# vaenyr/stable-diffusion-on-device

Measured on AMD Instinct MI355X. Metric: images/sec + per-UNet-step ms, SD v1.4 512x512 20-step PLMS, 1/2/4/8 MI355X, higher is better.
Workload: dtype f16; 1 GPU; SD v1.4 txt2img 512x512, 20-step PLMS (21 UNet evals, batch 2 = cond+uncond per image), CLIP encode + VAE decode + uint8, guidance 7.5; images_per_gpu=1, global_batch=1, parallelism=dp1 (image shards, 1 RCCL broadcast), hip_graph=True, trajectory_graph=True, decode_overlaps_next_sampling=False

## Files before the change

include/sdod_hip.h:

```cpp
#ifndef SDOD_HIP_H
#define SDOD_HIP_H

#include <stddef.h>
#include <stdint.h>

#ifndef SDOD_API
#define SDOD_API
#endif

#ifdef __cplusplus
extern "C" {
#endif

enum sdod_act { SDOD_ACT_NONE = 0, SDOD_ACT_SILU = 1, SDOD_ACT_GELU = 2, SDOD_ACT_QUICK_GELU = 3 };
enum sdod_dtype { SDOD_F16 = 0, SDOD_F32 = 1, SDOD_U8Q = 2, SDOD_BF16 = 3  };
enum sdod_a_mode { SDOD_A_ROWS = 0, SDOD_A_CONV3X3 = 1  };

typedef struct sdod_gemm_desc {
    const void* a;
    const void* a2;
    const void* w;
    const void* bias;
    const void* row_bias;
    const void* residual;
// ... 71 lines not shown
    size_t slab_floats;
    const void* bias;
    const void* bias2;
    const void* row_bias;
    int ld_row_bias;
    const void* residual;
    int ldr;
    void* x_out;
    float alpha;
    int act;
    int M, N;
} sdod_gn_reduce;
SDOD_API int sdod_gemm_reduce_info(const sdod_gemm_desc* d, sdod_gn_reduce* out);
SDOD_API int sdod_group_norm_reduce_ok(int hw, int c0, int c1, int groups);
SDOD_API int sdod_group_norm_reduce_nhwc(const sdod_gn_reduce* red, const void* x2, void* y, const float* weight,
                                         const float* bias, int n, int hw, int c0, int c1, int groups, float eps, int silu,
                                         void* stream);

SDOD_API int sdod_ln_fold_f16(void* w, int n, int k, int ldw, const float* gamma, const float* beta, const float* bias_in,
                              float* s_out, float* t_out, void* stream);
SDOD_API int sdod_compose_linear_f16(const void* p, int ldp, const void* w, int ldw, void* c, int ldc, int n_out, int n_mid, int k,
                                     const float* bias_w, const float* bias_p, float* bias_out, void* stream);
SDOD_API int sdod_layer_norm_f16(const void* x, void* y, const float* weight, const float* bias, int m, int c,
                                 float eps, void* stream);

SDOD_API int sdod_attention_f16(const void* q, const void* k, const void* v, void* out, int batch, int heads,
                                int lq, int lk, int d, int ldq, int ldk, int ldv, int ldo, float scale, int causal,
                                void* stream);

SDOD_API int sdod_xattn_fold_f16(const void* kv, int ld_kv, int k_off, int v_off, int n_img, int L, const void* wq, int ldq,
                                 const void* sq, const void* tq, const void* wo, int ldwo, int heads, int d, float scale, void* w1,
                                 void* s1, void* t1, void* w2, void* stream);

SDOD_API int sdod_softmax_rows_f16(const void* x, void* y, int m, int n, void* stream);

SDOD_API int sdod_geglu_f16(const void* x, void* y, int m, int c, void* stream);
SDOD_API int sdod_act_f16(const void* x, void* y, size_t n, int act, void* stream);
SDOD_API int sdod_add_f16(const void* a, const void* b, void* y, size_t n, void* stream);
SDOD_API int sdod_concat_channels_f16(const void* a, const void* b, void* y, size_t rows, int c0, int c1, void* stream);
SDOD_API int sdod_im2col3x3_small_f16(const void* x, void* y, int n_img, int h, int w, int c, int kpad, void* stream);
SDOD_API int sdod_latent_im2col_f16(const float* x, void* y, int n_img, int h, int w, int c, int kpad, float scale, void* stream);

SDOD_API int sdod_conv_in_f16(const float* x, const void* w, const float* bias, void* y, int n_img, int h, int wd, int c, int cout,
                              float scale, void* stream);
SDOD_API int sdod_image_conv_in_f16(const uint8_t* img, const void* w, const float* bias, void* y, int n_img, int h, int wd, int cout,
                                    void* stream);
SDOD_API int sdod_encode_latent_f32(const float* moments, const float* n1, const float* n2, float* x, float* z0, int n, int c, int hw,
                                    float sqrt_at, float sqrt_one_minus_at, uint64_t seed, uint64_t image_index0, void* stream);
SDOD_API int sdod_nchw_f32_to_nhwc_f16(const float* x, void* y, int n, int c, int hw, float scale, void* stream);
SDOD_API int sdod_latent_prep_f16(const float* x, const float* w, const float* b, void* y, int n, int c, int hw,
                                  float scale, void* stream);
SDOD_API int sdod_nhwc_f16_to_nchw_f32(const void* x, float* y, int n, int c, int hw, void* stream);
SDOD_API int sdod_embedding_f16(const int32_t* ids, const void* table, const void* pos, void* y, int rows, int seq,
                                int c, void* stream);
SDOD_API int sdod_timestep_features_f16(const float* t, void* y, int n, int dim, void* stream);

SDOD_API int sdod_stage_unet_inputs(const float* x, float* x_dst, size_t lat_count, int reps, const void* temb_row,
                                    void* temb_dst, size_t temb_width, int temb_reps, void* stream);
SDOD_API int sdod_randn_f32(float* out, uint32_t* words_out, size_t count, uint64_t seed, uint64_t stream_id, void* stream);

SDOD_API int sdod_cfg_combine(const void* eps_nhwc, float* e_out, int n, int c, int hw, float guidance,
                              int uncond_first, int mode, void* stream);
SDOD_API int sdod_dpm_update(float* x, const float* eps, float* y_prev, size_t count, int order, float sigma_s,
                             float alpha_s, float sigma_ratio, float c_prev, float c_cur, void* stream);
SDOD_API int sdod_ddim_step_f32(float* x, const float* e, size_t count, float sqrt_one_minus_at, float sqrt_at,
                                float sqrt_a_prev, float dir_coef, void* stream);
// ... 40 lines not shown
```

stable-diffusion-on-device_amd/csrc/gemm.hip:

```cpp
#include "common.h"
#include "sdod_hip.h"
#include "host_util.h"

#include <algorithm>
#include <cmath>
#include <cstdlib>
#include <type_traits>

namespace {

struct GemmP {
    const f16* a0;
    const f16* a1;
    const f16* w;
    const float* bias;
    const f16* row_bias;
    const f16* residual;
    f16* out;
    float* partial;
    int M, N, K;
    int lda, ldw, ldo, ldr;
    int mode;
    int h_in, w_in, h_out, w_out, c0, c1, stride, ups, ksize;
    int pad;
// ... 1131 lines not shown
                            acc[i][j][r] = e;
                            sum += e;
                        }
                    sum = quad_rows_sum(sum);
                    const float inv = __builtin_amdgcn_rcpf(sum);
#pragma unroll
                    for (int j = 0; j < TN; ++j)
#pragma unroll
                        for (int r = 0; r < 4; ++r) acc[i][j][r] *= inv;
                }
            }
        }
#pragma unroll
        for (int i = 0; i < TM; ++i) {
            const int ml = wm * WTM + i * 16 + e_m;
#pragma unroll
            for (int j = 0; j < TN; ++j) {
                const int nl = wn * WTN + j * 16 + e_n;
                f16x4 h;
#pragma unroll
                for (int r = 0; r < 4; ++r) h[r] = (f16)acc[i][j][r];
                *reinterpret_cast<f16x4*>(sC + ml * SC + nl) = h;
            }
        }
    }
    __syncthreads();
    STAMP(3);

    store_phase();
#ifdef SDOD_GEMM_STAMP
    wait_vmcnt<0>();
    STAMP(4);
#endif
}

template <int BM, int BN, int WM, int WN, int STAGES>
__global__ __launch_bounds__(768) void gemm_apanel_kernel(const GemmP p, const f16* __restrict__ zeros) {
    constexpr int NL = 4;
    constexpr int WTM = BM / WM, WTN = BN / WN;
    constexpr int TM = WTM / 16, TN = WTN / 16;
    constexpr int A_LD = BM / (8 * NL), B_LD = BN / (8 * NL);
    constexpr int AHEAD = STAGES - 1;
    constexpr int ASLAB = BM * 64, WSLAB = BN * 64;
    static_assert(WM * WN == 4 && BM % 32 == 0 && BN % 64 == 0 && BN <= 128 && TM >= 1 && TN >= 2 && TN % 2 == 0, "tile shape");
    static_assert(B_LD * AHEAD + 2 < 64, "vmcnt is a 6-bit counter");

    extern __shared__ __attribute__((aligned(16))) char smem_raw[];
    const int KT = p.K / BK;
    f16* sAp = reinterpret_cast<f16*>(smem_raw);
    f16* sW = sAp + (size_t)KT * ASLAB;
    float* colv = reinterpret_cast<float*>(sW + (size_t)STAGES * WSLAB);
    float* ln_stats = colv + 6 * BN;

    const int tid = threadIdx.x;
    const int lane = tid & 63;
    const int wave = __builtin_amdgcn_readfirstlane(tid >> 6);

    const int lid = xcd_remap(blockIdx.x, (int)gridDim.x);
    int pm, ng;
    if (p.ap_nmajor) {
        ng = lid / p.ap_panels;
        pm = lid - ng * p.ap_panels;
    } else {
        pm = lid / p.ap_groups;
        ng = lid - pm * p.ap_groups;
    }
// ... 1759 lines not shown
    hipStream_t st = (hipStream_t)stream;
    int rc = sdod_gemm_f16(d, stream);
    if (rc) return rc;
    hipEvent_t ev[32];
    for (int i = 0; i < 2 * iters; ++i) SDOD_HIP_CHECK(hipEventCreate(&ev[i]));
    float* sink = (float*)scratch;
    const size_t a_bytes = d->a_mode == SDOD_A_ROWS ? (size_t)d->M * d->lda * 2 : (size_t)d->n_img * d->h_in * d->w_in * d->c0 * 2;
    for (int i = 0; i < iters; ++i) {
        SDOD_LAUNCH(cache_sweep_kernel, dim3(2048), dim3(256), 0, st, (float4*)scratch, scratch_bytes / 16);
        touch(d->a, a_bytes, sink, st);
        if (d->a2 && d->c1) touch(d->a2, (size_t)d->n_img * d->h_in * d->w_in * d->c1 * 2, sink, st);
        if (d->residual) touch(d->residual, (size_t)d->M * d->ldr * 2, sink, st);
        if (d->t0 && d->k_tail) touch(d->t0, (size_t)d->M * d->tc0 * 2, sink, st);
        if (d->t1 && d->k_tail && d->tc1) touch(d->t1, (size_t)d->M * d->tc1 * 2, sink, st);
        SDOD_HIP_CHECK(hipEventRecord(ev[2 * i], st));
        rc = sdod_gemm_f16(d, stream);
        if (rc) return rc;
        SDOD_HIP_CHECK(hipEventRecord(ev[2 * i + 1], st));
    }
    SDOD_HIP_CHECK(hipEventSynchronize(ev[2 * iters - 1]));
    float tot = 0.f, best = 1e30f;
    for (int i = 0; i < iters; ++i) {
        float ms = 0.f;
        SDOD_HIP_CHECK(hipEventElapsedTime(&ms, ev[2 * i], ev[2 * i + 1]));
        tot += ms;
        best = ms < best ? ms : best;
    }
    for (int i = 0; i < 2 * iters; ++i) (void)hipEventDestroy(ev[i]);
    *ms_avg = tot / iters;
    if (ms_min) *ms_min = best;
    return 0;
    SDOD_CATCH
}
```

stable-diffusion-on-device_amd/csrc/graphs.hip:

```cpp
#include "engine.h"

namespace sdod {

static void check_rc2(int rc) {
    if (rc != 0) throw Error(rc, get_last_error());
}

int Graph::group_first(const std::string& group) const {
    auto it = gindex_.find(group);
    if (it == gindex_.end()) throw Error(INTERNAL_ERROR, "unknown parameter group " + group);
    return groups_[it->second].front();
}

const char* Graph::group_base(const std::string& group) const {
    auto it = gindex_.find(group);
    if (it == gindex_.end()) throw Error(INTERNAL_ERROR, "unknown parameter group " + group);
    return params_[groups_[it->second].front()].dev;
}

Act Graph::res_block(const std::string& pfx, const Act& x, const Act* x2, int cout, const f16* emb_all, int emb_ld, int& emb_off) {
    const int cin = x.c + (x2 ? x2->c : 0);
    quant_rows(x.rows());
    const int n1w = P(pfx + ".in_layers.0.weight", {cin}, PK_VEC), n1b = P(pfx + ".in_layers.0.bias", {cin}, PK_VEC);
    const int c1w = P(pfx + ".in_layers.2.weight", {cout, cin, 3, 3}, PK_CONV3), c1b = P(pfx + ".in_layers.2.bias", {cout}, PK_VEC);
// ... 82 lines not shown
    const bool compose = compose_on && !quant_block;
    int f2w, pow_;
    if (compose) {
        f2w = Pc(tb + ".ff.net.2.weight", {C, 4 * C}, PK_LINEAR, 5 * C, 0, -1);
        pow_ = lin ? Pc(pfx + ".proj_out.weight", {C, C}, PK_LINEAR, 5 * C, 4 * C, f2w)
                   : Pc(pfx + ".proj_out.weight", {C, C, 1, 1}, PK_CONV1, 5 * C, 4 * C, f2w);
    } else {
        f2w = P(tb + ".ff.net.2.weight", {C, 4 * C}, PK_LINEAR);
        pow_ = lin ? P(pfx + ".proj_out.weight", {C, C}, PK_LINEAR) : P(pfx + ".proj_out.weight", {C, C, 1, 1}, PK_CONV1);
    }
    const int f2b = P(tb + ".ff.net.2.bias", {C}, PK_VEC);
    const int pob = P(pfx + ".proj_out.bias", {C}, PK_VEC);
    if (mode_ == DECLARE) return act(x.n, x.h, x.w, C);

    Act g = group_norm(x, nullptr, nw, nb, 1e-6f, false);
    Act t0 = act(B, 1, L, C);
    { GemmOpt o; o.bias = pib; linear(g.p, rows, C, piw, C, t0.p, o); }
    release(g);
    const bool fold = !quant_block;
    auto normed = [&](const Act& src, int lw, int lb) -> Act { return layer_norm(src, lw, lb, 1e-5f); };
    f16* qkv = alloc((size_t)rows * 3 * C);
    if (fold) {
        GemmOpt o; o.ln_w = l1w; o.ln_b = l1b;
        linear_raw(t0.p, rows, C, reinterpret_cast<const f16*>(group_base(gq)), C, 3 * C, qkv, o);
    } else {
        Act nrm = normed(t0, l1w, l1b);
        GemmOpt o; o.wq_scale = qscale_of(group_first(gq)); o.wq_off = qoff_of(group_first(gq));
        linear_raw(nrm.p, rows, C, reinterpret_cast<const f16*>(group_base(gq)), C, 3 * C, qkv, o);
        release(nrm);
    }
    f16* a1 = alloc((size_t)rows * C);
    attention(qkv, qkv + C, qkv + 2 * C, a1, B, heads, L, L, d, 3 * C, 3 * C, 3 * C, C, false);
    release(qkv);
    Act t1 = act(B, 1, L, C);
    { GemmOpt o; o.bias = o1b; o.residual = t0.p; linear(a1, rows, C, o1w, C, t1.p, o); }
    release(a1); release(t0);
    static const bool xfold_on = [] { const char* e = std::getenv("SDOD_XATTN_FOLD"); return !(e && e[0] == '0'); }();
    const int NK = heads * 80;
    const bool xfold = xfold_on && fold && ctx.w <= 80 && NK % 320 == 0 && L % 32 == 0 && d <= 160 && d % 4 == 0;
    if (xfold) {
        f16 *w1 = nullptr, *w2 = nullptr;
        float *s1 = nullptr, *t1v = nullptr;
        f16* wq = reinterpret_cast<f16*>(params_[q2w].dev);
        const f16* wo = reinterpret_cast<const f16*>(params_[o2w].dev);
        if (mode_ == REAL) {
            SDOD_HIP_CHECK(hipMalloc((void**)&w1, (size_t)B * NK * C * sizeof(f16)));
            SDOD_HIP_CHECK(hipMalloc((void**)&w2, (size_t)B * NK * C * sizeof(f16)));
            SDOD_HIP_CHECK(hipMalloc((void**)&s1, (size_t)B * NK * sizeof(float)));
            SDOD_HIP_CHECK(hipMalloc((void**)&t1v, (size_t)B * NK * sizeof(float)));
            derived_.push_back(w1); derived_.push_back(w2); derived_.push_back(s1); derived_.push_back(t1v);
            const LnVecs qv = ln_fold_vectors(wq, C, C, C, l2w, l2b, nullptr);
            const f16* kvp = kv_all_;
            const int ldkv = kv_total_, koff = my_kv, Lk = ctx.w, hh = heads, dd = d;
            const float scale = 1.0f / sqrtf((float)d);
            to_static_ = true;
            sink().push_back(Op{[=](hipStream_t st) {
                check_rc2(sdod_xattn_fold_f16(kvp, ldkv, koff, koff + C, B, Lk, wq, C, qv.s, qv.t, wo, C, hh, dd, scale, w1, s1, t1v, w2, st));
            }, "xattn_fold", 4.0 * B * NK * (double)C * d, 4.0 * B * NK * C * 2, "C" + std::to_string(C) + " d" + std::to_string(d)});
            to_static_ = false;
        }
        const f16* w1p = mode_ == REAL ? w1 : wq;
        const f16* w2p = mode_ == REAL ? w2 : wq;
        f16* pb = alloc((size_t)rows * NK);
        { GemmOpt o; o.ln_s_raw = mode_ == REAL ? s1 : reinterpret_cast<const float*>(wq); o.bias_raw = mode_ == REAL ? t1v : reinterpret_cast<const float*>(wq);
          o.w_img_stride = NK * C; o.vec_img_stride = NK; o.softmax_cols = 80; o.rows_per_img = L;
          linear_raw(t1.p, rows, C, w1p, C, NK, pb, o); }
        GemmOpt o2;
        o2.bias = o2b; o2.residual = t1.p; o2.w_img_stride = C * NK; o2.rows_per_img = L;
        if (compose) {
            f16* cat = alloc((size_t)rows * 5 * C);
            f16* t2c = cat + 4 * C;
            o2.ldr = C; o2.ldo = 5 * C;
            linear_raw(pb, rows, NK, w2p, NK, C, t2c, o2);
            release(pb); release(t1);
            { GemmOpt o; o.bias = f1b; o.geglu = true; o.ln_w = l3w; o.ln_b = l3b; o.lda = 5 * C; o.ldo = 5 * C; linear(t2c, rows, C, f1w, 8 * C, cat, o); }
            float* bc = nullptr;
            if (mode_ == REAL) {
                SDOD_HIP_CHECK(hipMalloc((void**)&bc, (size_t)C * sizeof(float)));
                derived_.push_back(bc);
                f16* wc = reinterpret_cast<f16*>(params_[f2w].dev);
                compose_jobs_.push_back(ComposeJob{wc, wc + 4 * C, 5 * C, C, C, 4 * C, W<float>(f2b), W<float>(pob), bc});
            }
            Act out = act(x.n, x.h, x.w, C);
            { GemmOpt o; o.bias_raw = mode_ == REAL ? bc : reinterpret_cast<const float*>(params_[f2w].dev); o.residual = x.p;
              linear_raw(cat, rows, 5 * C, reinterpret_cast<const f16*>(params_[f2w].dev), 5 * C, C, out.p, o); }
            release(cat);
            return out;
        }
        Act t2 = act(B, 1, L, C);
        linear_raw(pb, rows, NK, w2p, NK, C, t2.p, o2);
        release(pb); release(t1);
        f16* gg = alloc((size_t)rows * 4 * C);
        { GemmOpt o; o.bias = f1b; o.geglu = true; o.ln_w = l3w; o.ln_b = l3b; linear(t2.p, rows, C, f1w, 8 * C, gg, o); }
        Act t3 = act(B, 1, L, C);
        { GemmOpt o; o.bias = f2b; o.residual = t2.p; linear(gg, rows, 4 * C, f2w, C, t3.p, o); }
        release(gg); release(t2);
        Act out = act(x.n, x.h, x.w, C);
        { GemmOpt o; o.bias = pob; o.residual = x.p; linear(t3.p, rows, C, pow_, C, out.p, o); }
        release(t3);
        return out;
    }
    f16* q2 = alloc((size_t)rows * C);
    if (fold) {
        GemmOpt o; o.ln_w = l2w; o.ln_b = l2b; linear(t1.p, rows, C, q2w, C, q2, o);
    } else {
        Act nrm = normed(t1, l2w, l2b);
        linear(nrm.p, rows, C, q2w, C, q2, GemmOpt{});
        release(nrm);
    }
    const int Lk = ctx.w;
    const f16* kv = kv_all_ + my_kv;
    f16* a2 = alloc((size_t)rows * C);
    attention(q2, kv, kv + C, a2, B, heads, L, Lk, d, C, kv_total_, kv_total_, C, false);
    release(q2);
    if (compose) {
        f16* cat = alloc((size_t)rows * 5 * C);
        f16* t2c = cat + 4 * C;
        { GemmOpt o; o.bias = o2b; o.residual = t1.p; o.ldr = C; o.ldo = 5 * C; linear(a2, rows, C, o2w, C, t2c, o); }
        release(a2); release(t1);
        { GemmOpt o; o.bias = f1b; o.geglu = true; o.ln_w = l3w; o.ln_b = l3b; o.lda = 5 * C; o.ldo = 5 * C; linear(t2c, rows, C, f1w, 8 * C, cat, o); }
        float* bc = nullptr;
        if (mode_ == REAL) {
            SDOD_HIP_CHECK(hipMalloc((void**)&bc, (size_t)C * sizeof(float)));
            derived_.push_back(bc);
            f16* wc = reinterpret_cast<f16*>(params_[f2w].dev);
            compose_jobs_.push_back(ComposeJob{wc, wc + 4 * C, 5 * C, C, C, 4 * C, W<float>(f2b), W<float>(pob), bc});
        }
        Act out = act(x.n, x.h, x.w, C);
        { GemmOpt o; o.bias_raw = mode_ == REAL ? bc : reinterpret_cast<const float*>(params_[f2w].dev); o.residual = x.p;
          linear_raw(cat, rows, 5 * C, reinterpret_cast<const f16*>(params_[f2w].dev), 5 * C, C, out.p, o); }
        release(cat);
        return out;
    }
    Act t2 = act(B, 1, L, C);
    { GemmOpt o; o.bias = o2b; o.residual = t1.p; linear(a2, rows, C, o2w, C, t2.p, o); }
    release(a2); release(t1);
    f16* gg = alloc((size_t)rows * 4 * C);
    if (fold) {
        GemmOpt o; o.bias = f1b; o.geglu = true; o.ln_w = l3w; o.ln_b = l3b; linear(t2.p, rows, C, f1w, 8 * C, gg, o);
    } else {
        Act nrm = normed(t2, l3w, l3b);
        GemmOpt o; o.bias = f1b; o.geglu = true; linear(nrm.p, rows, C, f1w, 8 * C, gg, o);
        release(nrm);
    }
    Act t3 = act(B, 1, L, C);
    { GemmOpt o; o.bias = f2b; o.residual = t2.p; linear(gg, rows, 4 * C, f2w, C, t3.p, o); }
    release(gg); release(t2);
    Act out = act(x.n, x.h, x.w, C);
    { GemmOpt o; o.bias = pob; o.residual = x.p; linear(t3.p, rows, C, pow_, C, out.p, o); }
    release(t3);
    return out;
}

void Graph::build_unet() {
    const int B = batch_, H = cfg_.latent_h, Wd = cfg_.latent_w, LC = cfg_.latent_channels;
    const int MC = cfg_.model_channels, EC = 4 * MC, cd = cfg_.context_dim, CL = cfg_.context_len;
    SDOD_REQUIRE(LC * 9 <= 64, "latent_channels too large for the small-Cin path");
    const int mult[4] = {1, 2, 4, 4};

    if (mode_ != DECLARE) {
        int tot = 0;
        for (auto& rb : unet_res_blocks()) tot += rb.second;
        emb_total_ = tot;
    }
    float* x_in = (float*)io_alloc(inputs_, (size_t)B * LC * H * Wd * sizeof(float));
// ... 413 lines not shown
```

stable-diffusion-on-device_amd/sdod/amd/_lib.py:

```python
import ctypes
import os

_HERE = os.path.dirname(os.path.abspath(__file__))
LIB_DIR = os.path.normpath(os.path.join(_HERE, '..', '..', 'lib'))

_cache = {}


def load(name):
    if name in _cache:
        return _cache[name]
    path = os.path.join(LIB_DIR, os.environ.get('SDOD_LIBSDOD', name) if name == 'libsdod.so' else name)
    if not os.path.exists(path):
        raise ImportError(
            f'{path} not found: build the MI355X extension first '
            f'(python -c "import __graft_entry__ as g; g.build()" or make -C stable-diffusion-on-device_amd). '
            f'There is no CPU fallback for the HIP path.')
    lib = ctypes.CDLL(path, mode=ctypes.RTLD_GLOBAL)
    _cache[name] = lib
    return lib


class SdodError(RuntimeError):
    def __init__(self, code, msg):
# ... 48 lines not shown
def _declare(lib):
    P = c_void_p
    sig = {
        'sdod_gemm_f16': (c_int, [ctypes.POINTER(GemmDesc), P]),
        'sdod_gemm_fixup': (c_int, [P]),
        'sdod_gemm_fixup_counters': (c_size_t, []),
        'sdod_gemm_workspace_bytes': (c_size_t, [ctypes.POINTER(GemmDesc)]),
        'sdod_gemm_plan': (c_int, [ctypes.POINTER(GemmDesc), ctypes.POINTER(c_int), ctypes.POINTER(c_int)]),
        'sdod_gemm_halo_ok': (c_int, [ctypes.POINTER(GemmDesc), c_int]),
        'sdod_gemm_panel_ok': (c_int, [ctypes.POINTER(GemmDesc), c_int]),
        'sdod_gemm_xcd_panels': (c_int, [ctypes.POINTER(GemmDesc)]),
        'sdod_gemm_time': (c_int, [ctypes.POINTER(GemmDesc), P, c_int, ctypes.POINTER(c_float)]),
        'sdod_gemm_time_cold': (c_int, [ctypes.POINTER(GemmDesc), P, c_int, P, c_size_t, ctypes.POINTER(c_float), ctypes.POINTER(c_float)]),
        'sdod_gemm_num_tiles': (c_int, []),
        'sdod_gemm_tile_info': (c_int, [c_int, ctypes.POINTER(c_int)]),
        'sdod_gemm_tile_shape': (c_int, [c_int, ctypes.POINTER(c_int), ctypes.POINTER(c_int), ctypes.POINTER(c_int)]),
        'sdod_gemm_reduce_info': (c_int, [ctypes.POINTER(GemmDesc), P]),
        'sdod_group_norm_reduce_ok': (c_int, [c_int, c_int, c_int, c_int]),
        'sdod_group_norm_reduce_nhwc': (c_int, [P, P, P, P, P, c_int, c_int, c_int, c_int, c_int, c_float, c_int, P]),
        'sdod_group_norm_launches': (c_int, [c_int, c_int, c_int, c_int]),
        'sdod_group_norm_workspace_bytes': (c_size_t, [c_int, c_int]),
        'sdod_group_norm_layout': (c_int, [c_int, c_int] + [ctypes.POINTER(c_size_t)] * 5),
        'sdod_group_norm_status': (c_int, []),
        'sdod_group_norm_clear_error': (c_int, []),
        'sdod_group_norm_path': (c_int, [c_int, c_int, c_int, c_int, c_int, c_int]),
        'sdod_group_norm_nchw_workspace_bytes': (c_size_t, [c_int, c_int]),
        'sdod_group_norm_nchw': (c_int, [P, P, P, P, c_int, c_int, ctypes.c_longlong, c_int, c_float, c_int, c_int, P, P]),
        'sdod_group_norm_nhwc': (c_int, [P, P, P, P, P, c_int, c_int, c_int, c_int, c_int, c_float, c_int, c_int, P, P]),
        'sdod_layer_norm_f16': (c_int, [P, P, P, P, c_int, c_int, c_float, P]),
        'sdod_ln_fold_f16': (c_int, [P, c_int, c_int, c_int, P, P, P, P, P, P]),
        'sdod_compose_linear_f16': (c_int, [P, c_int, P, c_int, P, c_int, c_int, c_int, c_int, P, P, P, P]),
        'sdod_attention_f16': (c_int, [P, P, P, P, c_int, c_int, c_int, c_int, c_int, c_int, c_int, c_int, c_int, c_float, c_int, P]),
        'sdod_xattn_fold_f16': (c_int, [P, c_int, c_int, c_int, c_int, c_int, P, c_int, P, P, P, c_int, c_int, c_int, c_float, P, P, P, P, P]),
        'sdod_softmax_rows_f16': (c_int, [P, P, c_int, c_int, P]),
        'sdod_geglu_f16': (c_int, [P, P, c_int, c_int, P]),
        'sdod_act_f16': (c_int, [P, P, c_size_t, c_int, P]),
        'sdod_add_f16': (c_int, [P, P, P, c_size_t, P]),
        'sdod_concat_channels_f16': (c_int, [P, P, P, c_size_t, c_int, c_int, P]),
        'sdod_im2col3x3_small_f16': (c_int, [P, P, c_int, c_int, c_int, c_int, c_int, P]),
        'sdod_latent_im2col_f16': (c_int, [P, P, c_int, c_int, c_int, c_int, c_int, c_float, P]),
        'sdod_conv_in_f16': (c_int, [P, P, P, P, c_int, c_int, c_int, c_int, c_int, c_float, P]),
        'sdod_image_conv_in_f16': (c_int, [P, P, P, P, c_int, c_int, c_int, c_int, P]),
        'sdod_encode_latent_f32': (c_int, [P, P, P, P, P, c_int, c_int, c_int, c_float, c_float, ctypes.c_uint64, ctypes.c_uint64, P]),
        'sdod_plms_update': (c_int, [ctypes.POINTER(PlmsUpdateArgs), P]),
        'sdod_dpm_step': (c_int, [ctypes.POINTER(DpmStepArgs), P]),
        'sdod_nchw_f32_to_nhwc_f16': (c_int, [P, P, c_int, c_int, c_int, c_float, P]),
        'sdod_nhwc_f16_to_nchw_f32': (c_int, [P, P, c_int, c_int, c_int, P]),
        'sdod_latent_prep_f16': (c_int, [P, P, P, P, c_int, c_int, c_int, c_float, P]),
        'sdod_embedding_f16': (c_int, [P, P, P, P, c_int, c_int, c_int, P]),
        'sdod_timestep_features_f16': (c_int, [P, P, c_int, c_int, P]),
        'sdod_stage_unet_inputs': (c_int, [P, P, c_size_t, c_int, P, P, c_size_t, c_int, P]),
        'sdod_randn_f32': (c_int, [P, P, c_size_t, ctypes.c_uint64, ctypes.c_uint64, P]),
        'sdod_cfg_combine': (c_int, [P, P, c_int, c_int, c_int, c_float, c_int, c_int, P]),
        'sdod_dpm_update': (c_int, [P, P, P, c_size_t, c_int, c_float, c_float, c_float, c_float, c_float, P]),
        'sdod_ddim_step_f32': (c_int, [P, P, c_size_t, c_float, c_float, c_float, c_float, P]),
        'sdod_lincomb4_f32': (c_int, [P, P, P, P, P, c_float, c_float, c_float, c_float, c_float, c_size_t, P]),
        'sdod_image_to_u8': (c_int, [P, P, c_size_t, c_float, c_float, c_int, P]),
        'sdod_hip_last_error': (c_char_p, []),
        'sdod_hip_device_info': (c_int, [ctypes.POINTER(c_int), ctypes.POINTER(c_size_t), c_char_p, c_int]),
    }
    for name, (res, args) in sig.items():
        fn = getattr(lib, name)
        fn.restype = res
        fn.argtypes = args


HIP_SYMBOLS = [
    'sdod_gemm_f16', 'sdod_gemm_fixup', 'sdod_gemm_fixup_counters', 'sdod_gemm_workspace_bytes', 'sdod_gemm_plan', 'sdod_gemm_halo_ok', 'sdod_gemm_panel_ok', 'sdod_gemm_xcd_panels', 'sdod_gemm_num_tiles', 'sdod_gemm_tile_shape', 'sdod_gemm_tile_info', 'sdod_gemm_time', 'sdod_gemm_time_cold', 'sdod_group_norm_workspace_bytes', 'sdod_group_norm_layout', 'sdod_group_norm_status', 'sdod_group_norm_clear_error', 'sdod_l2_prefetch', 'sdod_group_norm_launches', 'sdod_group_norm_path', 'sdod_group_norm_nhwc', 'sdod_group_norm_nchw', 'sdod_group_norm_nchw_workspace_bytes', 'sdod_gemm_reduce_info', 'sdod_group_norm_reduce_ok', 'sdod_group_norm_reduce_nhwc',
    'sdod_layer_norm_f16', 'sdod_ln_fold_f16', 'sdod_compose_linear_f16', 'sdod_attention_f16', 'sdod_xattn_fold_f16', 'sdod_softmax_rows_f16', 'sdod_geglu_f16', 'sdod_act_f16',
    'sdod_add_f16', 'sdod_concat_channels_f16', 'sdod_im2col3x3_small_f16', 'sdod_latent_im2col_f16', 'sdod_conv_in_f16', 'sdod_image_conv_in_f16', 'sdod_encode_latent_f32', 'sdod_plms_update', 'sdod_dpm_step', 'sdod_nchw_f32_to_nhwc_f16',
    'sdod_nhwc_f16_to_nchw_f32', 'sdod_latent_prep_f16', 'sdod_embedding_f16', 'sdod_timestep_features_f16', 'sdod_cfg_combine', 'sdod_stage_unet_inputs', 'sdod_randn_f32',
    'sdod_dpm_update', 'sdod_ddim_step_f32', 'sdod_lincomb4_f32', 'sdod_image_to_u8', 'sdod_hip_last_error',
    'sdod_hip_device_info',
]


def check(code):
    if code != 0:
        msg = hip().sdod_hip_last_error()
        raise SdodError(code, msg.decode() if msg else 'unknown error')
```

stable-diffusion-on-device_amd/sdod/amd/ops.py:

```python
import ctypes

import torch

from . import _lib
from ._lib import GemmDesc, check

ACT = {None: 0, 'none': 0, 'silu': 1, 'gelu': 2, 'quick_gelu': 3}


def _stream():
    return ctypes.c_void_p(torch.cuda.current_stream().cuda_stream)


def _p(t):
    return None if t is None else ctypes.c_void_p(t.data_ptr())


def _req(t, dtype=None, name='tensor'):
    if not t.is_cuda:
        raise ValueError(f'{name} must live on the GPU')
    if not t.is_contiguous():
        raise ValueError(f'{name} must be contiguous')
    if dtype is not None and t.dtype != dtype:
        raise ValueError(f'{name} must be {dtype}, got {t.dtype}')
# ... 230 lines not shown


def attention(q, k, v, heads, scale=None, causal=False, out=None):
    lib = _lib.hip()
    for t, nme in ((q, 'q'), (k, 'k'), (v, 'v')):
        _req(t, torch.float16, nme)
    b, lq, c = q.shape
    lk = k.shape[1]
    d = c // heads
    if scale is None:
        scale = d ** -0.5
    if out is None:
        out = torch.empty_like(q)
    check(lib.sdod_attention_f16(_p(q), _p(k), _p(v), _p(out), b, heads, lq, lk, d, q.shape[2], k.shape[2], v.shape[2],
                                 out.shape[2], scale, 1 if causal else 0, _stream()))
    return out


def xattn_fold(kv, k_off, v_off, n_img, L, wq, sq, tq, wo, heads, scale=None):
    lib = _lib.hip()
    _req(kv, torch.float16, 'kv'); _req(wq, torch.float16, 'wq'); _req(wo, torch.float16, 'wo')
    _req(sq, torch.float32, 'sq'); _req(tq, torch.float32, 'tq')
    c = wq.shape[0]; d = c // heads
    if scale is None:
        scale = d ** -0.5
    w1 = torch.empty(n_img, heads * 80, c, dtype=torch.float16, device=kv.device)
    w2 = torch.empty(n_img, c, heads * 80, dtype=torch.float16, device=kv.device)
    s1 = torch.empty(n_img, heads * 80, dtype=torch.float32, device=kv.device); t1 = torch.empty_like(s1)
    check(lib.sdod_xattn_fold_f16(_p(kv), kv.shape[-1], k_off, v_off, n_img, L, _p(wq), wq.shape[1], _p(sq), _p(tq), _p(wo), wo.shape[1],
                                  heads, d, scale, _p(w1), _p(s1), _p(t1), _p(w2), _stream()))
    return w1, s1, t1, w2


def attention_strided(q, k, v, out, batch, heads, lq, lk, d, ldq, ldk, ldv, ldo, scale, causal=False):
    lib = _lib.hip()
    check(lib.sdod_attention_f16(q, k, v, out, batch, heads, lq, lk, d, ldq, ldk, ldv, ldo, scale, 1 if causal else 0,
                                 _stream()))


def softmax_rows(x, out=None):
    lib = _lib.hip()
    _req(x, torch.float16, 'x')
    n = x.shape[-1]; m = x.numel() // n
    if out is None:
        out = torch.empty_like(x)
    check(lib.sdod_softmax_rows_f16(_p(x), _p(out), m, n, _stream()))
    return out


def geglu(x, out=None):
    lib = _lib.hip()
    _req(x, torch.float16, 'x')
    c = x.shape[-1] // 2; m = x.numel() // (2 * c)
    if out is None:
        out = torch.empty(x.shape[:-1] + (c,), dtype=torch.float16, device=x.device)
    check(lib.sdod_geglu_f16(_p(x), _p(out), m, c, _stream()))
    return out


def activation(x, act, out=None):
    lib = _lib.hip()
    _req(x, torch.float16, 'x')
    if out is None:
        out = torch.empty_like(x)
    check(lib.sdod_act_f16(_p(x), _p(out), x.numel(), ACT[act], _stream()))
    return out
# ... 230 lines not shown
```

Measured before the change: 10.67 images/s.

## Fuse self-attn out-proj, folded cross-attn and out-proj into one chain kernel

Adds a persistent kernel for C=320 transformer blocks. It chains four stages per 32-row tile while keeping the intermediates in LDS: the attention output projection with residual, the LayerNorm-folded cross-attention score GEMM with per-head softmax, the P·W2 projection, and the bias plus residual. Producer waves stream weight slices into an LDS ring through async DMA, and an optional L2 prefetch of per-image weights runs alongside. The goal is to remove three GEMM launches and their HBM round trips for t1 and the score buffer. The cost is lower parallelism, since each block recomputes a full 320/640-wide reduction chain, plus a fixed, shape-specialised path that only applies to the 64x64 resolution level.

```diff
diff --git a/include/sdod_hip.h b/include/sdod_hip.h
--- a/include/sdod_hip.h
+++ b/include/sdod_hip.h
@@ -127,6 +127,11 @@
                                  const void* sq, const void* tq, const void* wo, int ldwo, int heads, int d, float scale, void* w1,
                                  void* s1, void* t1, void* w2, void* stream);
 
+SDOD_API int sdod_xattn_chain_f16(const void* a1, const void* t0, const void* wo1, const float* bo1, const void* w1, const float* s1,
+                                  const float* t1v, const void* w2, const float* bo2, int M, int rows_per_img, void* out, int ldo,
+                                  void* t1_out, void* p_out, void* stream);
+SDOD_API int sdod_xattn_chain_ok(int c, int heads, int score_cols, int rows_per_img);
+
 SDOD_API int sdod_softmax_rows_f16(const void* x, void* y, int m, int n, void* stream);
 
 SDOD_API int sdod_geglu_f16(const void* x, void* y, int m, int c, void* stream);
diff --git a/stable-diffusion-on-device_amd/csrc/gemm.hip b/stable-diffusion-on-device_amd/csrc/gemm.hip
--- a/stable-diffusion-on-device_amd/csrc/gemm.hip
+++ b/stable-diffusion-on-device_amd/csrc/gemm.hip
@@ -1187,6 +1187,301 @@
     wait_vmcnt<0>();
     STAMP(4);
 #endif
+}
+
+namespace chain {
+constexpr int C = 320, NK = 640, BM = 32, HALF = 160, NSLOT = 5, AHEAD = NSLOT - 1;
+constexpr int NL = 4, NC = 4;
+constexpr int LOADS = HALF * 64 * 2 / 1024 / NL;
+constexpr int STEPS = 5 * 10;
+constexpr int SLOT = HALF * 64;
+constexpr int ABLK = BM * C;
+constexpr int PF_BYTES = NL * 64 * 4;
+constexpr size_t SMEM = (size_t)(NSLOT * SLOT + 2 * ABLK) * sizeof(f16) + (size_t)BM * 2 * sizeof(float) + PF_BYTES;
+static_assert(LOADS * (AHEAD - 1) < 64, "vmcnt is a 6-bit counter");
+static_assert(SMEM <= 160 * 1024, "LDS");
+}
+
+struct ChainP {
+    const f16* a1;
+    const f16* t0;
+    const f16* wo1;
+    const float* bo1;
+    const f16* w1;
+    const float* s1;
+    const float* t1v;
+    const f16* w2;
+    const float* bo2;
+    f16* out;
+    f16* t1_out;
+    f16* p_out;
+    int M, ldo, K;
+    float alpha, ln_eps;
+    unsigned mg_rpi, sh_rpi;
+    int pf_parts;
+};
+
+__global__ __launch_bounds__(512) void xattn_chain_kernel(const ChainP p) {
+    using namespace chain;
+    extern __shared__ __attribute__((aligned(16))) char smem_raw[];
+    f16* ring = reinterpret_cast<f16*>(smem_raw);
+    f16* t1s = ring + NSLOT * SLOT;
+    f16* ps = t1s + ABLK;
+    float* stats = reinterpret_cast<float*>(ps + ABLK);
+
+    const int tid = threadIdx.x, lane = tid & 63;
+    const int wave = __builtin_amdgcn_readfirstlane(tid >> 6);
+    const int lid = xcd_remap(blockIdx.x, gridDim.x);
+    const int m0 = lid * BM;
+    const int img = fast_div(m0, p.mg_rpi, p.sh_rpi);
+    const f16* w1 = p.w1 + (size_t)img * NK * C;
+    const f16* w2 = p.w2 + (size_t)img * C * NK;
+    const int lrow = lane >> 3, lchunk = (lane & 7) ^ lrow;
+
+    if (wave >= NC) {
+        const int lw = wave - NC;
+        unsigned off320[LOADS], off640[LOADS];
+#pragma unroll
+        for (int i = 0; i < LOADS; ++i) {
+            const unsigned r = (unsigned)((i * NL + lw) * 8 + lrow);
+            off320[i] = (r * 320u + (unsigned)lchunk * 8u) * 2u;
+            off640[i] = (r * 640u + (unsigned)lchunk * 8u) * 2u;
+        }
+        if (p.pf_parts > 0) {
+            constexpr int LINES = STEPS * HALF;
+            const int q = lid % p.pf_parts, per = (LINES + p.pf_parts - 1) / p.pf_parts;
+            const int end = min(LINES, (q + 1) * per);
+            for (int k = 0; k * NL * 64 < per; ++k) {
+                int line = q * per + k * NL * 64 + lw * 64 + lane;
+                line = line < end ? line : q * per;
+                const int s = line / HALF, r = line - s * HALF;
+                const int blk = s / 10, w = s - blk * 10, kt = w >> 1, h = w & 1;
+                const f16* g = blk == 2 || blk == 4 ? w2 + (size_t)(h * HALF + r) * NK + (blk == 4 ? C : 0) + kt * 64
+                             : blk == 0 ? p.wo1 + (size_t)(h * HALF + r) * C + kt * 64
+                                        : w1 + (size_t)((blk == 3 ? C : 0) + h * HALF + r) * C + kt * 64;
+                __builtin_amdgcn_global_load_lds((glb_void_ptr)g, (lds_void_ptr)(reinterpret_cast<char*>(stats + 2 * BM) + lw * 256), 4, 0, 0);
+            }
+        }
+        {
+            const f16* ab = p.a1 + (size_t)(m0 + lw * 8) * C;
+            const unsigned off = (unsigned)(lrow * C + lchunk * 8) * 2u;
+#pragma unroll
+            for (int kt = 0; kt < 5; ++kt) lds_dma16_saddr(ab + kt * 64, off, ps + kt * BM * 64 + lw * 8 * 64);
+        }
+        auto issue = [&](int s) {
+            const int blk = s / 10, w = s - blk * 10, kt = w >> 1, h = w & 1;
+            f16* dst = ring + (s % NSLOT) * SLOT;
+            if (blk == 2 || blk == 4) {
+                const f16* base = w2 + (size_t)(h * HALF) * NK + (blk == 4 ? C : 0) + kt * 64;
+#pragma unroll
+                for (int i = 0; i < LOADS; ++i) lds_dma16_saddr(base, off640[i], dst + (i * NL + lw) * 8 * 64);
+            } else {
+                const f16* base = blk == 0 ? p.wo1 + (size_t)(h * HALF) * C + kt * 64 : w1 + (size_t)((blk == 3 ? C : 0) + h * HALF) * C + kt * 64;
+#pragma unroll
+                for (int i = 0; i < LOADS; ++i) lds_dma16_saddr(base, off320[i], dst + (i * NL + lw) * 8 * 64);
+            }
+        };
+#pragma unroll
+        for (int s = 0; s < AHEAD; ++s) issue(s);
+        for (int s = 0; s < STEPS; ++s) {
+            wait_younger<LOADS, AHEAD - 1>(STEPS - 1 - s);
+            __builtin_amdgcn_s_barrier();
+            if (s + AHEAD < STEPS) issue(s + AHEAD);
+        }
+        return;
+    }
+
+    const int cw = wave;
+    const int frag_row = lane & 15, frag_chunk = lane >> 4;
+    const int e_m = lane & 15, e_n = (lane >> 4) * 4;
+    f16x4 res0[2][5];
+#pragma unroll
+    for (int i = 0; i < 2; ++i)
+#pragma unroll
+        for (int j = 0; j < 5; ++j)
+            res0[i][j] = *reinterpret_cast<const f16x4*>(p.t0 + (size_t)(m0 + i * 16 + e_m) * C + cw * 80 + j * 16 + e_n);
+
+    f32x4 acc[2][5], acco[2][5];
+    auto zero_acc = [](f32x4 (&a)[2][5]) {
+#pragma unroll
+        for (int i = 0; i < 2; ++i)
+#pragma unroll
+            for (int j = 0; j < 5; ++j) a[i][j] = f32x4{0.f, 0.f, 0.f, 0.f};
+    };
+    zero_acc(acc);
+    zero_acc(acco);
+    auto aoff = [](int row, int col) { return (col >> 6) * (BM * 64) + lds_off(row, (col & 63) >> 3) + (col & 7); };
+
+    int slot = 0;
+    auto run_block = [&](f32x4 (&a)[2][5], const f16* aop, bool stats_first) {
+        for (int kt = 0; kt < 5; ++kt) {
+#pragma unroll
+            for (int h = 0; h < 2; ++h) {
+                __syncthreads();
+                if (stats_first && kt == 0 && h == 0) {
+                    float r1 = 0.f, r2 = 0.f;
+#pragma unroll
+                    for (int k = 0; k < 5; ++k) {
+                        const f16x8 v = *reinterpret_cast<const f16x8*>(t1s + k * BM * 64 + cw * 8 * 64 + lane * 8);
+                        const f16x2 one2 = {(f16)1.0f, (f16)1.0f};
+#pragma unroll
+                        for (int e = 0; e < 8; e += 2) {
+                            const f16x2 pr = {v[e], v[e + 1]};
+                            r1 = __builtin_amdgcn_fdot2(pr, one2, r1, false);
+                            r2 = __builtin_amdgcn_fdot2(pr, pr, r2, false);
+                        }
+                    }
+                    r1 = oct_sum(r1);
+                    r2 = oct_sum(r2);
+                    if ((lane & 7) == 0) {
+                        const float mean = r1 / (float)p.K;
+                        float var = r2 / (float)p.K - mean * mean;
+                        var = var < 0.f ? 0.f : var;
+                        const int r = cw * 8 + lrow;
+                        stats[2 * r] = mean;
+                        stats[2 * r + 1] = rsqrt_fast(var + p.ln_eps);
+                    }
+                }
+                if ((cw >> 1) == h) {
+                    const f16* sA = aop + kt * BM * 64;
+                    const f16* sB = ring + slot * SLOT + (cw & 1) * 80 * 64;
+                    f16x8 xa[2][2], wb[2][5];
+#pragma unroll
+                    for (int ks = 0; ks < 2; ++ks) {
+#pragma unroll
+                        for (int i = 0; i < 2; ++i) xa[ks][i] = *reinterpret_cast<const f16x8*>(sA + lds_off(i * 16 + frag_row, ks * 4 + frag_chunk));
+#pragma unroll
+                        for (int j = 0; j < 5; ++j) wb[ks][j] = *reinterpret_cast<const f16x8*>(sB + lds_off(j * 16 + frag_row, ks * 4 + frag_chunk));
+                    }
+                    __builtin_amdgcn_s_setprio(1);
+#pragma unroll
+                    for (int ks = 0; ks < 2; ++ks)
+#pragma unroll
+                        for (int j = 0; j < 5; ++j)
+#pragma unroll
+                            for (int i = 0; i < 2; ++i) a[i][j] = mfma16(wb[ks][j], xa[ks][i], a[i][j]);
+                    __builtin_amdgcn_s_setprio(0);
+                }
+                slot = slot + 1 == NSLOT ? 0 : slot + 1;
+            }
+        }
+    };
+
+    auto score_epilogue = [&](int round) {
+        const int hd = round * 4 + cw;
+        const float* s1 = p.s1 + (size_t)img * NK + hd * 80;
+        const float* tv = p.t1v + (size_t)img * NK + hd * 80;
+        const float alpha = p.alpha;
+#pragma unroll
+        for (int i = 0; i < 2; ++i) {
+            const int ml = i * 16 + e_m;
+            const float mean = stats[2 * ml], rstd = stats[2 * ml + 1];
+#pragma unroll
+            for (int j = 0; j < 5; ++j) {
+                const f32x4 sv = *reinterpret_cast<const f32x4*>(s1 + j * 16 + e_n);
+#pragma unroll
+                for (int r = 0; r < 4; ++r) acc[i][j][r] = rstd * (acc[i][j][r] * alpha - mean * sv[r]);
+            }
+        }
+#pragma unroll
+        for (int j = 0; j < 5; ++j) {
+            const f32x4 b1 = *reinterpret_cast<const f32x4*>(tv + j * 16 + e_n);
+#pragma unroll
+            for (int i = 0; i < 2; ++i)
+#pragma unroll
+                for (int r = 0; r < 4; ++r) acc[i][j][r] = acc[i][j][r] + b1[r];
+        }
+#pragma unroll
+        for (int i = 0; i < 2; ++i) {
+            float mx = acc[i][0][0];
+#pragma unroll
+            for (int j = 0; j < 5; ++j)
+#pragma unroll
+                for (int r = 0; r < 4; ++r) mx = fmaxf(mx, acc[i][j][r]);
+            mx = quad_rows_max(mx);
+            float sum = 0.f;
+#pragma unroll
+            for (int j = 0; j < 5; ++j)
+#pragma unroll
+                for (int r = 0; r < 4; ++r) {
+                    const float e = __builtin_amdgcn_exp2f(acc[i][j][r] - mx);
+                    acc[i][j][r] = e;
+                    sum += e;
+                }
+            sum = quad_rows_sum(sum);
+            const float inv = __builtin_amdgcn_rcpf(sum);
+            const int ml = i * 16 + e_m;
+#pragma unroll
+            for (int j = 0; j < 5; ++j) {
+                f16x4 hv;
+#pragma unroll
+                for (int r = 0; r < 4; ++r) hv[r] = (f16)(acc[i][j][r] * inv);
+                const int col = cw * 80 + j * 16 + e_n;
+                *reinterpret_cast<f16x4*>(ps + aoff(ml, col)) = hv;
+                if (p.p_out != nullptr) *reinterpret_cast<f16x4*>(p.p_out + (size_t)(m0 + ml) * NK + round * C + col) = hv;
+            }
+        }
+        zero_acc(acc);
+    };
+
+    run_block(acc, ps, false);
+    {
+        const float* b = p.bo1 + cw * 80;
+#pragma unroll
+        for (int j = 0; j < 5; ++j) {
+            const f32x4 b1 = *reinterpret_cast<const f32x4*>(b + j * 16 + e_n);
+#pragma unroll
+            for (int i = 0; i < 2; ++i) {
+                const int ml = i * 16 + e_m, col = cw * 80 + j * 16 + e_n;
+                f16x4 hv;
+#pragma unroll
+                for (int r = 0; r < 4; ++r) hv[r] = (f16)((float)(f16)(acc[i][j][r] + b1[r]) + (float)res0[i][j][r]);
+                *reinterpret_cast<f16x4*>(t1s + aoff(ml, col)) = hv;
+                if (p.t1_out != nullptr) *reinterpret_cast<f16x4*>(p.t1_out + (size_t)(m0 + ml) * C + col) = hv;
+            }
+        }
+        zero_acc(acc);
+    }
+    run_block(acc, t1s, true);
+    score_epilogue(0);
+    run_block(acco, ps, false);
+    run_block(acc, t1s, false);
+    score_epilogue(1);
+    run_block(acco, ps, false);
+
+    {
+        const float* b = p.bo2 + cw * 80;
+#pragma unroll
+        for (int j = 0; j < 5; ++j) {
+            const f32x4 b1 = *reinterpret_cast<const f32x4*>(b + j * 16 + e_n);
+#pragma unroll
+            for (int i = 0; i < 2; ++i) {
+                const int o = aoff(i * 16 + e_m, cw * 80 + j * 16 + e_n);
+                const f16x4 rr = *reinterpret_cast<const f16x4*>(t1s + o);
+                f16x4 hv;
+#pragma unroll
+                for (int r = 0; r < 4; ++r) hv[r] = (f16)((float)(f16)(acco[i][j][r] + b1[r]) + (float)rr[r]);
+                *reinterpret_cast<f16x4*>(t1s + o) = hv;
+            }
+        }
+#pragma unroll
+        for (int k = 0; k < 5; ++k) {
+            const int idx = lane + 64 * k, row = idx / 10, seg = idx - row * 10;
+            const int col = cw * 80 + seg * 8;
+            stg8(p.out + (size_t)(m0 + row) * p.ldo + col, *reinterpret_cast<const f16x8*>(t1s + aoff(row, col)));
+        }
+    }
+}
+
+hipError_t launch_xattn_chain(const ChainP& p, int blocks, hipStream_t st) {
+    static std::atomic<unsigned long long> attr_devs{0};
+    if (sdod::first_use_on_device(attr_devs)) {
+        hipError_t e = hipFuncSetAttribute(reinterpret_cast<const void*>(&xattn_chain_kernel), hipFuncAttributeMaxDynamicSharedMemorySize,
+                                           (int)chain::SMEM);
+        if (e != hipSuccess) return e;
+    }
+    SDOD_LAUNCH(xattn_chain_kernel, dim3(blocks), dim3(512), chain::SMEM, st, p);
+    return hipGetLastError();
 }
 
 template <int BM, int BN, int WM, int WN, int STAGES>
@@ -3012,3 +3307,33 @@
     return 0;
     SDOD_CATCH
 }
+
+extern "C" int sdod_xattn_chain_ok(int c, int heads, int score_cols, int rows_per_img) {
+    return c == chain::C && heads * score_cols == chain::NK && score_cols == 80 && rows_per_img > 0 && rows_per_img % chain::BM == 0;
+}
+
+extern "C" int sdod_xattn_chain_f16(const void* a1, const void* t0, const void* wo1, const float* bo1, const void* w1, const float* s1,
+                                    const float* t1v, const void* w2, const float* bo2, int M, int rows_per_img, void* out, int ldo,
+                                    void* t1_out, void* p_out, void* stream) {
+    SDOD_TRY
+    SDOD_REQUIRE(a1 && t0 && wo1 && bo1 && w1 && s1 && t1v && w2 && bo2 && out, "null pointer");
+    SDOD_REQUIRE(M > 0 && rows_per_img > 0 && rows_per_img % chain::BM == 0 && M % rows_per_img == 0,
+                 "rows_per_img must be a positive multiple of 32 and divide M");
+    SDOD_REQUIRE(ldo >= chain::C && ldo % 8 == 0, "ldo must be >= 320 and a multiple of 8");
+    const uintptr_t al = (uintptr_t)a1 | (uintptr_t)t0 | (uintptr_t)wo1 | (uintptr_t)bo1 | (uintptr_t)w1 | (uintptr_t)s1 |
+                         (uintptr_t)t1v | (uintptr_t)w2 | (uintptr_t)bo2 | (uintptr_t)out | (uintptr_t)t1_out | (uintptr_t)p_out;
+    SDOD_REQUIRE((al & 15) == 0, "operands must be 16-byte aligned");
+    ChainP p{};
+    p.a1 = (const f16*)a1; p.t0 = (const f16*)t0; p.wo1 = (const f16*)wo1; p.bo1 = bo1;
+    p.w1 = (const f16*)w1; p.s1 = s1; p.t1v = t1v; p.w2 = (const f16*)w2; p.bo2 = bo2;
+    p.out = (f16*)out; p.t1_out = (f16*)t1_out; p.p_out = (f16*)p_out;
+    p.M = M; p.ldo = ldo; p.K = chain::C;
+    p.alpha = 1.0f; p.ln_eps = 1e-5f;
+    make_magic((unsigned)rows_per_img, &p.mg_rpi, &p.sh_rpi);
+    static const bool l2pf = [] { const char* e = std::getenv("SDOD_XATTN_CHAIN_L2PF"); return !(e && e[0] == '0'); }();
+    const int blocks = M / chain::BM;
+    p.pf_parts = l2pf ? std::max(1, std::min(32, blocks / 8)) : 0;
+    SDOD_HIP_CHECK(launch_xattn_chain(p, blocks, (hipStream_t)stream));
+    return 0;
+    SDOD_CATCH
+}
diff --git a/stable-diffusion-on-device_amd/csrc/graphs.hip b/stable-diffusion-on-device_amd/csrc/graphs.hip
--- a/stable-diffusion-on-device_amd/csrc/graphs.hip
+++ b/stable-diffusion-on-device_amd/csrc/graphs.hip
@@ -138,12 +138,32 @@
     f16* a1 = alloc((size_t)rows * C);
     attention(qkv, qkv + C, qkv + 2 * C, a1, B, heads, L, L, d, 3 * C, 3 * C, 3 * C, C, false);
     release(qkv);
-    Act t1 = act(B, 1, L, C);
-    { GemmOpt o; o.bias = o1b; o.residual = t0.p; linear(a1, rows, C, o1w, C, t1.p, o); }
-    release(a1); release(t0);
     static const bool xfold_on = [] { const char* e = std::getenv("SDOD_XATTN_FOLD"); return !(e && e[0] == '0'); }();
     const int NK = heads * 80;
     const bool xfold = xfold_on && fold && ctx.w <= 80 && NK % 320 == 0 && L % 32 == 0 && d <= 160 && d % 4 == 0;
+    static const bool chain_on = [] { const char* e = std::getenv("SDOD_XATTN_CHAIN"); return !(e && e[0] == '0'); }();
+    const bool xchain = chain_on && xfold && compose && sdod_xattn_chain_ok(C, heads, 80, L) && params_[o1w].ld <= 0;
+    Act t1;
+    if (!xchain) {
+        t1 = act(B, 1, L, C);
+        { GemmOpt o; o.bias = o1b; o.residual = t0.p; linear(a1, rows, C, o1w, C, t1.p, o); }
+        release(a1); release(t0);
+    }
+    auto composed_tail = [&](f16* cat, f16* t2c) -> Act {
+        { GemmOpt o; o.bias = f1b; o.geglu = true; o.ln_w = l3w; o.ln_b = l3b; o.lda = 5 * C; o.ldo = 5 * C; linear(t2c, rows, C, f1w, 8 * C, cat, o); }
+        float* bc = nullptr;
+        if (mode_ == REAL) {
+            SDOD_HIP_CHECK(hipMalloc((void**)&bc, (size_t)C * sizeof(float)));
+            derived_.push_back(bc);
+            f16* wc = reinterpret_cast<f16*>(params_[f2w].dev);
+            compose_jobs_.push_back(ComposeJob{wc, wc + 4 * C, 5 * C, C, C, 4 * C, W<float>(f2b), W<float>(pob), bc});
+        }
+        Act out = act(x.n, x.h, x.w, C);
+        { GemmOpt o; o.bias_raw = mode_ == REAL ? bc : reinterpret_cast<const float*>(params_[f2w].dev); o.residual = x.p;
+          linear_raw(cat, rows, 5 * C, reinterpret_cast<const f16*>(params_[f2w].dev), 5 * C, C, out.p, o); }
+        release(cat);
+        return out;
+    };
     if (xfold) {
         f16 *w1 = nullptr, *w2 = nullptr;
         float *s1 = nullptr, *t1v = nullptr;
@@ -167,6 +187,27 @@
         }
         const f16* w1p = mode_ == REAL ? w1 : wq;
         const f16* w2p = mode_ == REAL ? w2 : wq;
+        if (xchain) {
+            f16* cat = alloc((size_t)rows * 5 * C);
+            f16* t2c = cat + 4 * C;
+            if (mode_ == REAL) {
+                const f16* a1p = a1; const f16* t0p = t0.p;
+                const f16* wo1 = reinterpret_cast<const f16*>(params_[o1w].dev);
+                const float *bo1 = W<float>(o1b), *bo2 = W<float>(o2b);
+                const int M = rows, rpi = L;
+                const double fl = 2.0 * rows * C * ((double)C + 2.0 * NK);
+                flops_ += fl;
+                settle();
+                sink().push_back(Op{[=](hipStream_t st) {
+                    check_rc2(sdod_xattn_chain_f16(a1p, t0p, wo1, bo1, w1, s1, t1v, w2, bo2, M, rpi, t2c, 5 * C, nullptr, nullptr, st));
+                }, "xattn_chain", fl, 3.0 * rows * C * 2 + (double)C * C * 2 + 4.0 * B * NK * C, "rows M" + std::to_string(rows) + " C" + std::to_string(C) +
+                   " NK" + std::to_string(NK) + " x1"});
+            } else {
+                settle();
+            }
+            release(a1); release(t0);
+            return composed_tail(cat, t2c);
+        }
         f16* pb = alloc((size_t)rows * NK);
         { GemmOpt o; o.ln_s_raw = mode_ == REAL ? s1 : reinterpret_cast<const float*>(wq); o.bias_raw = mode_ == REAL ? t1v : reinterpret_cast<const float*>(wq);
           o.w_img_stride = NK * C; o.vec_img_stride = NK; o.softmax_cols = 80; o.rows_per_img = L;
@@ -179,19 +220,7 @@
             o2.ldr = C; o2.ldo = 5 * C;
             linear_raw(pb, rows, NK, w2p, NK, C, t2c, o2);
             release(pb); release(t1);
-            { GemmOpt o; o.bias = f1b; o.geglu = true; o.ln_w = l3w; o.ln_b = l3b; o.lda = 5 * C; o.ldo = 5 * C; linear(t2c, rows, C, f1w, 8 * C, cat, o); }
-            float* bc = nullptr;
-            if (mode_ == REAL) {
-                SDOD_HIP_CHECK(hipMalloc((void**)&bc, (size_t)C * sizeof(float)));
-                derived_.push_back(bc);
-                f16* wc = reinterpret_cast<f16*>(params_[f2w].dev);
-                compose_jobs_.push_back(ComposeJob{wc, wc + 4 * C, 5 * C, C, C, 4 * C, W<float>(f2b), W<float>(pob), bc});
-            }
-            Act out = act(x.n, x.h, x.w, C);
-            { GemmOpt o; o.bias_raw = mode_ == REAL ? bc : reinterpret_cast<const float*>(params_[f2w].dev); o.residual = x.p;
-              linear_raw(cat, rows, 5 * C, reinterpret_cast<const f16*>(params_[f2w].dev), 5 * C, C, out.p, o); }
-            release(cat);
-            return out;
+            return composed_tail(cat, t2c);
         }
         Act t2 = act(B, 1, L, C);
         linear_raw(pb, rows, NK, w2p, NK, C, t2.p, o2);
@@ -224,19 +253,7 @@
         f16* t2c = cat + 4 * C;
         { GemmOpt o; o.bias = o2b; o.residual = t1.p; o.ldr = C; o.ldo = 5 * C; linear(a2, rows, C, o2w, C, t2c, o); }
         release(a2); release(t1);
-        { GemmOpt o; o.bias = f1b; o.geglu = true; o.ln_w = l3w; o.ln_b = l3b; o.lda = 5 * C; o.ldo = 5 * C; linear(t2c, rows, C, f1w, 8 * C, cat, o); }
-        float* bc = nullptr;
-        if (mode_ == REAL) {
-            SDOD_HIP_CHECK(hipMalloc((void**)&bc, (size_t)C * sizeof(float)));
-            derived_.push_back(bc);
-            f16* wc = reinterpret_cast<f16*>(params_[f2w].dev);
-            compose_jobs_.push_back(ComposeJob{wc, wc + 4 * C, 5 * C, C, C, 4 * C, W<float>(f2b), W<float>(pob), bc});
-        }
-        Act out = act(x.n, x.h, x.w, C);
-        { GemmOpt o; o.bias_raw = mode_ == REAL ? bc : reinterpret_cast<const float*>(params_[f2w].dev); o.residual = x.p;
-          linear_raw(cat, rows, 5 * C, reinterpret_cast<const f16*>(params_[f2w].dev), 5 * C, C, out.p, o); }
-        release(cat);
-        return out;
+        return composed_tail(cat, t2c);
     }
     Act t2 = act(B, 1, L, C);
     { GemmOpt o; o.bias = o2b; o.residual = t1.p; linear(a2, rows, C, o2w, C, t2.p, o); }
diff --git a/stable-diffusion-on-device_amd/sdod/amd/_lib.py b/stable-diffusion-on-device_amd/sdod/amd/_lib.py
--- a/stable-diffusion-on-device_amd/sdod/amd/_lib.py
+++ b/stable-diffusion-on-device_amd/sdod/amd/_lib.py
@@ -104,6 +104,8 @@
         'sdod_compose_linear_f16': (c_int, [P, c_int, P, c_int, P, c_int, c_int, c_int, c_int, P, P, P, P]),
         'sdod_attention_f16': (c_int, [P, P, P, P, c_int, c_int, c_int, c_int, c_int, c_int, c_int, c_int, c_int, c_float, c_int, P]),
         'sdod_xattn_fold_f16': (c_int, [P, c_int, c_int, c_int, c_int, c_int, P, c_int, P, P, P, c_int, c_int, c_int, c_float, P, P, P, P, P]),
+        'sdod_xattn_chain_f16': (c_int, [P, P, P, P, P, P, P, P, P, c_int, c_int, P, c_int, P, P, P]),
+        'sdod_xattn_chain_ok': (c_int, [c_int, c_int, c_int, c_int]),
         'sdod_softmax_rows_f16': (c_int, [P, P, c_int, c_int, P]),
         'sdod_geglu_f16': (c_int, [P, P, c_int, c_int, P]),
         'sdod_act_f16': (c_int, [P, P, c_size_t, c_int, P]),
@@ -139,7 +141,7 @@
 
 HIP_SYMBOLS = [
     'sdod_gemm_f16', 'sdod_gemm_fixup', 'sdod_gemm_fixup_counters', 'sdod_gemm_workspace_bytes', 'sdod_gemm_plan', 'sdod_gemm_halo_ok', 'sdod_gemm_panel_ok', 'sdod_gemm_xcd_panels', 'sdod_gemm_num_tiles', 'sdod_gemm_tile_shape', 'sdod_gemm_tile_info', 'sdod_gemm_time', 'sdod_gemm_time_cold', 'sdod_group_norm_workspace_bytes', 'sdod_group_norm_layout', 'sdod_group_norm_status', 'sdod_group_norm_clear_error', 'sdod_l2_prefetch', 'sdod_group_norm_launches', 'sdod_group_norm_path', 'sdod_group_norm_nhwc', 'sdod_group_norm_nchw', 'sdod_group_norm_nchw_workspace_bytes', 'sdod_gemm_reduce_info', 'sdod_group_norm_reduce_ok', 'sdod_group_norm_reduce_nhwc',
-    'sdod_layer_norm_f16', 'sdod_ln_fold_f16', 'sdod_compose_linear_f16', 'sdod_attention_f16', 'sdod_xattn_fold_f16', 'sdod_softmax_rows_f16', 'sdod_geglu_f16', 'sdod_act_f16',
+    'sdod_layer_norm_f16', 'sdod_ln_fold_f16', 'sdod_compose_linear_f16', 'sdod_attention_f16', 'sdod_xattn_fold_f16', 'sdod_xattn_chain_f16', 'sdod_xattn_chain_ok', 'sdod_softmax_rows_f16', 'sdod_geglu_f16', 'sdod_act_f16',
     'sdod_add_f16', 'sdod_concat_channels_f16', 'sdod_im2col3x3_small_f16', 'sdod_latent_im2col_f16', 'sdod_conv_in_f16', 'sdod_image_conv_in_f16', 'sdod_encode_latent_f32', 'sdod_plms_update', 'sdod_dpm_step', 'sdod_nchw_f32_to_nhwc_f16',
     'sdod_nhwc_f16_to_nchw_f32', 'sdod_latent_prep_f16', 'sdod_embedding_f16', 'sdod_timestep_features_f16', 'sdod_cfg_combine', 'sdod_stage_unet_inputs', 'sdod_randn_f32',
     'sdod_dpm_update', 'sdod_ddim_step_f32', 'sdod_lincomb4_f32', 'sdod_image_to_u8', 'sdod_hip_last_error',
diff --git a/stable-diffusion-on-device_amd/sdod/amd/ops.py b/stable-diffusion-on-device_amd/sdod/amd/ops.py
--- a/stable-diffusion-on-device_amd/sdod/amd/ops.py
+++ b/stable-diffusion-on-device_amd/sdod/amd/ops.py
@@ -286,6 +286,23 @@
     return w1, s1, t1, w2
 
 
+def xattn_chain(a1, t0, wo1, bo1, w1, s1, t1v, w2, bo2, rows_per_img, out=None, stages=False):
+    lib = _lib.hip()
+    for t, n in ((a1, 'a1'), (t0, 't0'), (wo1, 'wo1'), (w1, 'w1'), (w2, 'w2')):
+        _req(t, torch.float16, n)
+    for t, n in ((bo1, 'bo1'), (s1, 's1'), (t1v, 't1v'), (bo2, 'bo2')):
+        _req(t, torch.float32, n)
+    m = a1.shape[0]
+    if out is None:
+        out = torch.empty(m, wo1.shape[0], dtype=torch.float16, device=a1.device)
+    assert out.stride(1) == 1 and out.shape[0] == m
+    t1 = torch.empty(m, 320, dtype=torch.float16, device=a1.device) if stages else None
+    p = torch.empty(m, 640, dtype=torch.float16, device=a1.device) if stages else None
+    check(lib.sdod_xattn_chain_f16(_p(a1), _p(t0), _p(wo1), _p(bo1), _p(w1), _p(s1), _p(t1v), _p(w2), _p(bo2), m, rows_per_img,
+                                   _p(out), out.stride(0), _p(t1) if stages else None, _p(p) if stages else None, _stream()))
+    return (out, t1, p) if stages else out
+
+
 def attention_strided(q, k, v, out, batch, heads, lq, lk, d, ldq, ldk, ldv, ldo, scale, causal=False):
     lib = _lib.hip()
     check(lib.sdod_attention_f16(q, k, v, out, batch, heads, lq, lk, d, ldq, ldk, ldv, ldo, scale, 1 if causal else 0,
```

New measurement: 10.79 images/s, median of 6. 1.01x the previous value.
